# jyf588/SimGAN

Measured on AMD Instinct MI355X. Metric: env-steps/sec of GAIL-dyn PPO update, higher is better.
Workload: dtype f32; 1 GPU; northstar: GAIL-dyn update, T=128 N=512/GPU obs=47 act=12 D-in=86 policy=mlp h64 D h100 ppo_epoch=10 num_mini_batch=1...; optimizer_steps_per_update=2720, parallelism=single GPU

## Files before the change

simgan_amd/_lib.py:

```python
import ctypes as C
import os

import numpy as np

_HERE = os.path.dirname(os.path.abspath(__file__))
LIB_PATH = os.path.join(_HERE, "libsimgan_hip.so")

c_float_p = C.POINTER(C.c_float)
c_i64_p = C.POINTER(C.c_int64)
c_double_p = C.POINTER(C.c_double)
c_u8_p = C.POINTER(C.c_uint8)
c_int_p = C.POINTER(C.c_int)
H = C.c_void_p

F_OBS, F_OBS_FEAT, F_ACTIONS, F_REWARDS, F_VALUE_PREDS, F_RETURNS, F_LOGP, F_MASKS, F_BAD_MASKS, \
    F_ADVANTAGES = range(10)
POLICY_MLP, POLICY_SPLIT, POLICY_GRU = 0, 1, 2
DIST_GAUSSIAN, DIST_CATEGORICAL, DIST_BERNOULLI = 0, 1, 2
CHAIN_INNER_FIRST, CHAIN_LEARNER_FIRST = 0, 1
PROF_DISC_CHAIN, PROF_DISC_WGRAD, PROF_PPO_FWD, PROF_PPO_BWD, PROF_PPO_REDUCE, PROF_RELABEL, PROF_PPO_ADAM = range(7)


class PPOConfig(C.Structure):
    _fields_ = [("clip_param", C.c_float), ("ppo_epoch", C.c_int), ("num_mini_batch", C.c_int),
# ... 100 lines not shown
    "sg_disc_set_expert": (C.c_int, [H, c_float_p, C.c_int64]),
    "sg_disc_update_gail_dyn": (C.c_int, [H, H, C.c_int, c_i64_p, C.c_int64, c_i64_p, C.c_int64, c_float_p, C.c_int64, C.c_uint64,
                                          c_float_p, c_int_p]),
    "sg_disc_update_rows": (C.c_int, [H, c_float_p, C.c_int64, C.c_int, C.c_int, c_i64_p, C.c_int64, c_i64_p, C.c_int64, c_float_p,
                                      C.c_int64, C.c_uint64, c_float_p, c_int_p]),
    "sg_disc_predict_reward": (C.c_int, [H, c_float_p, C.c_int, C.c_float, c_float_p, C.c_float, c_float_p, c_float_p]),
    "sg_disc_predict_prob": (C.c_int, [H, c_float_p, C.c_int, c_float_p]),
    "sg_disc_predict_reward_steps": (C.c_int, [H, H, C.c_float, C.c_float, c_float_p, c_float_p]),
    "sg_disc_grad_pen": (C.c_int, [H, c_float_p, c_float_p, c_float_p, C.c_int, C.c_uint64, c_float_p]),
    "sg_disc_last_draws": (C.c_int, [H, c_i64_p, c_i64_p, c_float_p, c_i64_p]),
    "sg_disc_reset_returns": (C.c_int, [H]),
    "sg_disc_get_returns": (C.c_int, [H, c_float_p, C.c_int, c_int_p]),
    "sg_disc_set_returns": (C.c_int, [H, c_float_p, C.c_int]),
    "sg_disc_relabel_rewards": (C.c_int, [H, H, C.c_float, C.c_float, c_double_p]),
    "sg_disc_relabel_rewards_auto": (C.c_int, [H, H, C.c_float, C.c_double, C.c_int]),
    "sg_disc_set_rms": (C.c_int, [H, c_double_p]),
    "sg_disc_get_scalars": (C.c_int, [H, c_double_p]),
    "sg_disc_diagnostics": (C.c_int, [H, H, C.c_int, c_double_p]),
    "sg_disc_diagnostics_fetch": (C.c_int, [H, C.c_int, c_double_p]),
    "sg_disc_diagnostics_world": (C.c_int, [H, H, C.c_int, c_double_p]),
    "sg_results_publish": (C.c_int, [H, H, H, C.c_int]),
    "sg_results_fetch": (C.c_int, [H, C.c_int, c_double_p]),
    "sg_ctx_profile": (C.c_int, [H, C.c_int]),
    "sg_ctx_profile_read": (C.c_int, [H, C.c_int, c_double_p, c_i64_p]),
    "sg_ctx_profile_reset": (C.c_int, [H]),
    "sg_host_alloc": (C.c_int, [C.c_int64, C.POINTER(C.c_void_p)]),
    "sg_host_free": (C.c_int, [C.c_void_p]),
    "sg_ctx_mark": (C.c_int, [H, c_int_p]),
    "sg_ctx_mark_elapsed": (C.c_int, [H, C.c_int, C.c_int, c_double_p]),
}

TEST_LIB_PATH = os.path.join(_HERE, "libsimgan_hip_test.so")
c_ll_p = C.POINTER(C.c_longlong)
TEST_PROTOTYPES = {
    "sg_test_last_error": (C.c_char_p, []),
    "sg_test_gemm": (C.c_int, [H, C.c_int, C.c_int, C.c_int, C.c_int, c_float_p, c_float_p, c_float_p]),
    "sg_test_gemm_bench": (C.c_int, [H, C.c_int, C.c_int, C.c_int, C.c_int, C.c_int, C.c_int, C.c_int, c_ll_p]),
    "sg_test_mfma_probe": (C.c_int, [H, C.c_int, c_float_p, c_float_p, c_float_p]),
    "sg_test_flag_probe": (C.c_int, [H, C.c_int, C.c_int, C.c_int, C.c_int, c_ll_p, c_float_p]),
    "sg_test_fetch_probe": (C.c_int, [H, C.c_int, C.c_int, C.c_int, c_ll_p]),
    "sg_test_pmc_calibrate": (C.c_int, [H, C.c_int64]),
    "sg_test_pstep_probe": (C.c_int, [H, C.c_int, C.c_int, C.c_int, C.c_int, C.c_int, c_ll_p, c_int_p]),
    "sg_test_graph_state": (C.c_int, [H, H, c_int_p]),
    "sg_test_disc_gathers": (C.c_int, [H, c_ll_p]),
    "sg_test_rng": (C.c_int, [H, C.c_int, C.c_int64, C.c_uint64, C.c_void_p]),
    "sg_test_rng_at": (C.c_int, [H, C.c_int, C.c_int64, C.c_uint64, C.c_uint64, C.c_uint64, C.c_void_p]),
    "sg_test_rng_host": (C.c_int, [C.c_int, C.c_int64, C.c_uint64, C.c_uint64, C.c_uint64, C.c_void_p]),
    "sg_test_kfac_eig": (C.c_int, [H, C.c_int, c_float_p, c_float_p, c_float_p, C.POINTER(C.c_int)]),
    "sg_test_acktr_noise": (C.c_int, [H, C.c_int64, C.c_uint64, C.c_int64, c_float_p]),
    "sg_test_raise_kfac_error": (C.c_int, [H]),
    "sg_test_tear_probe": (C.c_int, [H, C.c_int, C.c_int, C.c_int, c_ll_p]),
    "sg_test_raise_handoff_error": (C.c_int, [H, H]),
    "sg_test_squash": (C.c_int, [c_float_p, c_float_p, C.c_int64]),
}
_TEST_LIB = None

_LIB = None


class SimganHipError(RuntimeError):
    pass


def load():
    global _LIB
    if _LIB is not None:
        return _LIB
    if not os.path.exists(LIB_PATH):
        raise SimganHipError(
            f"{LIB_PATH} not found: the HIP extension is not built. There is no CPU fallback; "
            "run `make -C simgan_amd/csrc` (hipcc, gfx950).")
    lib = C.CDLL(LIB_PATH)
    for name, (res, args) in PROTOTYPES.items():
        fn = getattr(lib, name)
        fn.restype = res
        fn.argtypes = args
    _LIB = lib
    return lib


def check(rc):
    if rc != 0:
        raise SimganHipError(load().sg_last_error().decode(errors="replace"))


def load_test():
    global _TEST_LIB
    if _TEST_LIB is not None:
        return _TEST_LIB
    load()
    if not os.path.exists(TEST_LIB_PATH):
        raise SimganHipError(f"{TEST_LIB_PATH} not found: run `make -C simgan_amd/csrc`")
    lib = C.CDLL(TEST_LIB_PATH)
    for name, (res, args) in TEST_PROTOTYPES.items():
        fn = getattr(lib, name)
        fn.restype = res
        fn.argtypes = args
    _TEST_LIB = lib
    return lib


def check_test(rc):
    if rc != 0:
        raise SimganHipError(load_test().sg_test_last_error().decode(errors="replace"))


# ... 168 lines not shown
```

simgan_amd/csrc/sg_ppo.hip:

```cpp
#include <math.h>
#include <stdlib.h>
#include <string.h>

#include <algorithm>
#include <vector>

#include "sg_common.h"
#include "sg_rng.hpp"
#include "sg_ppo_kernels.hpp"
#include "sg_kfac_host.hpp"
#include "sg_gru_kernels.hpp"

__global__ void k_fill_perm(int64_t* perm, int64_t n, int half_bits, uint64_t key) {
    const int64_t i = (int64_t)blockIdx.x * blockDim.x + threadIdx.x;
    if (i < n) perm[i] = sg_perm_at(i, n, half_bits, key);
}

int sg_fill_perm(sg_ctx* ctx, int64_t* d_perm, int64_t n, uint64_t seed, uint64_t stream_id) {
    const uint64_t key = sg_key(seed, 0x5045524Dull, stream_id);
    hipLaunchKernelGGL(k_fill_perm, dim3((unsigned)((n + 255) / 256)), dim3(256), 0, ctx->stream, d_perm, n,
                       sg_perm_half_bits((uint64_t)n), key);
    SG_CHECK(hipGetLastError());
    return 0;
}
// ... 845 lines not shown
    pa.slabs = a->d_slabs; pa.slab_stride = slab_stride; pa.ldP = ldP;
    pa.st = reinterpret_cast<SgOptState*>(a->d_state); pa.G = G; pa.k1 = 0;
    pa.pair = a->d_pair; pa.Xm = nullptr; pa.MA = nullptr; pa.sym_c = 0.f;
    for (int t = 0; t < 3; ++t) { pa.H1[t] = hX; pa.H2[t] = hX; pa.OUT[t] = hX; }
    pa.X = hX;
    pa.DX[0] = gb + o_dxa; pa.DX[1] = gb + o_dxc;
    pa.wbuf_floats = gw ? 0 : max_trunk_floats(d);

    GruScanArgs tr;
    tr.sr = gb + o_sr; tr.sz = gb + o_sz; tr.sn = gb + o_sn; tr.shn = gb + o_shn; tr.hm = gb + o_hm;
    GruBwdArgs ba;
    ba.g = g; ba.W = pol->d_params + g.off; ba.dxa = gb + o_dxa; ba.dxc = gb + o_dxc; ba.dx_ld = d.ldO;
    ba.sr = tr.sr; ba.sz = tr.sz; ba.sn = tr.sn; ba.shn = tr.shn; ba.hm = tr.hm; ba.T = T; ba.n = per;
    ba.dgi = gb + o_dgi; ba.dgh = gb + o_dgh;
    GruWgradArgs wa;
    wa.g = g; wa.dgi = ba.dgi; wa.dgh = ba.dgh; wa.hm = tr.hm; wa.rows_p = rows_p; wa.KS = KS; wa.partial = gb + o_part;
    const bool gw_scan = sg_gru_force_gw() || sg_gru_scan_lds(g, false) > (size_t)ctx->lds_bytes - 1024 ||
                         sg_gru_bwd_lds(g, false) > (size_t)ctx->lds_bytes - 1024;
    const int n_tiles = (G3 / 16) * (g.Op / 16 + Hp / 16) + 2 * (G3 / 16);
    const size_t lds_b = bwd_lds(MT);
    SgOptState* st = reinterpret_cast<SgOptState*>(a->d_state);

    auto enqueue_steps = [&]() -> int {
        hipLaunchKernelGGL(k_opt_prepare_first, dim3(1), dim3(1), 0, ctx->stream, st);
        for (int e = 0; e < E; ++e) {
            ga.perm = a->d_perms + (size_t)e * N;
            hipLaunchKernelGGL(k_gru_epoch_gather<0>, dim3((unsigned)TN), dim3(64), 0, ctx->stream, ga);
            for (int k = 0; k < S; ++k) {
                const size_t rb = (size_t)k * mb;
                const float* xk = gb + o_x + rb * g.ldO;
                const float* mk = gb + o_mk + rb;
                SG_TRY(sg_gru_forward_launch(ctx, g, pol->d_params + g.off, xk, g.ldO, gb + o_h0 + (size_t)k * per * g.H, mk, T, per,
                                             gb + o_gi, hX, d.ldO, nullptr, &tr));
                pa.ACT = epACT + rb * d.A; pa.SC = epSC + rb;
                pa.k1 = e * S + k + 1;
                if (d.dist == SG_DIST_CATEGORICAL)
                    SG_TRY(ppo_launch(ctx, ppo_bwd_fused_cat_dx_family, "k_ppo_bwd_dist_dx (Categorical)", SG_PROF_PPO_BWD, MT, d, dim3(G, 2),
                                      lds_b, pa, gw));
                else if (d.dist == SG_DIST_BERNOULLI)
                    SG_TRY(ppo_launch(ctx, ppo_bwd_fused_ber_dx_family, "k_ppo_bwd_dist_dx (Bernoulli)", SG_PROF_PPO_BWD, MT, d, dim3(G, 2),
                                      lds_b, pa, gw));
                else
                    SG_TRY(ppo_launch(ctx, ppo_bwd_fused_dx_family, "k_ppo_bwd (fused, with d loss / d h)", SG_PROF_PPO_BWD, MT, d, dim3(G, 2),
                                      lds_b, pa, gw));
                SG_LAUNCH(ctx, SG_PROF_PPO_REDUCE, k_ppo_reduce, dim3(nblk_r), dim3(256), 0, a->d_slabs, G, slab_stride, d.total, a->d_grad,
                          a->d_part);
                ba.masks = mk;
                if (gw_scan) hipLaunchKernelGGL(k_gru_scan_bwd<true>, dim3((per + 15) / 16), dim3(256), sg_gru_bwd_lds(g, true), ctx->stream, ba);
                else hipLaunchKernelGGL(k_gru_scan_bwd<false>, dim3((per + 15) / 16), dim3(256), sg_gru_bwd_lds(g, false), ctx->stream, ba);
                wa.x = xk;
                hipLaunchKernelGGL(k_gru_wgrad<0>, dim3(n_tiles, KS), dim3(64), 0, ctx->stream, wa);
                hipLaunchKernelGGL(k_gru_reduce<0>, dim3(gblocks), dim3(256), 0, ctx->stream, wa.partial, KS, g.total, a->d_grad, d.total,
                                   a->d_part, nblk_r);
                SG_LAUNCH(ctx, SG_PROF_PPO_ADAM, k_ppo_adam, dim3(nblk), dim3(256), 0, pol->d_params, a->d_m, a->d_v, a->d_grad, a->d_part,
                          nblk_r + gblocks, tot_all, st, e * S + k + 1, a->cfg.eps, a->cfg.max_grad_norm, pa.inv_B, a->d_loss_acc);
            }
        }
        hipLaunchKernelGGL(k_opt_commit, dim3(1), dim3(1), 0, ctx->stream, st, E * S);
        SG_CHECK(hipGetLastError());
        return 0;
    };
    const bool use_graph = !ctx->profile && !sg_env_is_off("SG_PPO_GRAPH");
    uint32_t fbits[6];
    const float fv[6] = {a->cfg.clip_param, a->cfg.value_loss_coef, a->cfg.entropy_coef, a->cfg.eps, a->cfg.max_grad_norm, pa.inv_B};
    memcpy(fbits, fv, sizeof fbits);
    const uint64_t key[SG_GRAPH_KEY_WORDS] = {
            (uint64_t)(uintptr_t)a->d_slabs, (uint64_t)(uintptr_t)a->d_stacks, (uint64_t)(uintptr_t)a->d_perms,
            (uint64_t)(uintptr_t)r->d_field[SG_F_OBS], (uint64_t)(uintptr_t)r->d_field[SG_F_ACTIONS],
            (uint64_t)(uintptr_t)r->d_field[SG_F_RETURNS], (uint64_t)(uintptr_t)pol->d_params,
            (uint64_t)TN, ((uint64_t)E << 32) | (uint64_t)M, ((uint64_t)MT << 32) | (uint64_t)G,
            ((uint64_t)fbits[0] << 32) | fbits[1], ((uint64_t)fbits[2] << 32) | fbits[3],
            ((uint64_t)fbits[4] << 32) | fbits[5], (uint64_t)a->cfg.use_clipped_value_loss,
            (uint64_t)(uintptr_t)r->d_field[SG_F_LOGP],
            0x475255ull + (gw ? 8 : 0) + (gw_scan ? 16 : 0) + ((uint64_t)d.dist << 24) + ((uint64_t)N << 32),
            (uint64_t)(uintptr_t)a->d_gru, (uint64_t)(uintptr_t)a->d_h0 ^ ((uint64_t)(uintptr_t)r->d_field[SG_F_MASKS] << 1)};
    SG_TRY(sg_graph_run(ctx, &a->steps_graph, use_graph, key, enqueue_steps));
    SG_CHECK(hipGetLastError());
    a->opt_t += (int64_t)E * S;
    if (!out3) return 0;
    double acc[3];
    SG_TRY(sg_ctx_fetch_f64(ctx, a->d_loss_acc, acc, 3));
    const double nu = (double)E * M;
    for (int i = 0; i < 3; ++i) out3[i] = (float)(acc[i] / nu);
    return 0;
}

#define SG_CNN_MAX_MB 4096
static int cnn_ppo_update(sg_ppo* a, sg_rollout* r, const int64_t* perms, int64_t n_perms, uint64_t seed, float out3[3]) {
    sg_ctx* ctx = a->ctx;
    sg_policy* pol = a->policy;
    const SgPolicyDesc& d = pol->desc;
    const SgCnnDesc& c = pol->cnnd;
    SG_REQUIRE(r->O == d.O && r->A == d.A, "sg_ppo_update: rollout dims (obs %d, act %d) do not match the policy (%d, %d)", r->O, r->A,
               d.O, d.A);
    SG_REQUIRE(!(ctx->use_comm && ctx->world > 1), "sg_ppo_update: PPO on the CNN base runs on one rank (world %d)", ctx->world);
    const int64_t TN = (int64_t)r->T * r->N;
    const int M = a->cfg.num_mini_batch, E = a->cfg.ppo_epoch;
    SG_REQUIRE(TN >= M, "PPO requires the number of processes (%d) * number of steps (%d) = %lld to be greater than "
               "or equal to the number of PPO mini batches (%d).", r->N, r->T, (long long)TN, M);
    SG_REQUIRE(TN < (1ll << 30), "sg_ppo_update: rollout too large");
    const int mb = (int)(TN / M);
    SG_REQUIRE(mb <= SG_CNN_MAX_MB, "sg_ppo_update: a minibatch of %d rows on the CNN base exceeds %d (its activation stacks are "
               "158 KB per row): raise num_mini_batch", mb, SG_CNN_MAX_MB);
    if (perms) {
        SG_REQUIRE(n_perms == (int64_t)E * TN, "sg_ppo_update: perms holds %lld indices, %d epochs x %lld rows need %lld",
                   (long long)n_perms, E, (long long)TN, (long long)E * TN);
        for (int64_t i = 0; i < n_perms; ++i)
            SG_REQUIRE(perms[i] >= 0 && perms[i] < TN, "sg_ppo_update: perms[%lld] = %lld is outside [0, %lld)", (long long)i,
                       (long long)perms[i], (long long)TN);
    }
    SG_CHECK(hipSetDevice(ctx->device));
    SG_TRY(enqueue_adv_stats(ctx, r, a, false));
    SG_TRY(ensure_cap(ctx->stream, &a->d_perms, &a->perms_cap, (int64_t)E * TN));
    a->last_perm_count = (int64_t)E * TN;
    if (perms) {
        SG_CHECK(hipMemcpyAsync(a->d_perms, perms, sizeof(int64_t) * (size_t)E * TN, hipMemcpyHostToDevice, ctx->stream));
        if (!out3) SG_CHECK(hipStreamSynchronize(ctx->stream));
    } else {
        for (int e = 0; e < E; ++e) SG_TRY(sg_fill_perm(ctx, a->d_perms + (size_t)e * TN, TN, seed, (uint64_t)e * 2654435761ull));
    }
    const int hld = d.trunk[0].Pp > 16 ? d.trunk[0].Pp : 16;
    const size_t heads_f = 2 * (size_t)mb * hld, fwd_f = sg_cnn_fwd_floats(c, mb), bwd_f = sg_cnn_bwd_floats(c, mb);
    bool grew = false;
    SG_TRY(ensure_cap(ctx->stream, &a->d_stacks, &a->stacks_cap, heads_f + fwd_f + bwd_f, &grew));
    if (grew) a->cleared.mode = SG_LAYOUT_INVALID;
    float* heads = a->d_stacks;
    float* act = heads + heads_f;
    float* bwd = act + fwd_f;
    hipLaunchKernelGGL(k_zero_f64, dim3(1), dim3(64), 0, ctx->stream, a->d_loss_acc, 4);
    const float inv_B = 1.0f / (float)mb;
    const int nblk = (c.total + 255) / 256;
    SgOptState* st = reinterpret_cast<SgOptState*>(a->d_state);
    const float* obs = r->d_field[SG_F_OBS];

    auto enqueue_steps = [&]() -> int {
        hipLaunchKernelGGL(k_opt_prepare_first, dim3(1), dim3(1), 0, ctx->stream, st);
        for (int e = 0; e < E; ++e)
            for (int k = 0; k < M; ++k) {
                const int64_t* idx = a->d_perms + (size_t)e * TN + (size_t)k * mb;
                SG_TRY(sg_cnn_forward_launch(ctx, pol, obs, idx, mb, act, heads, hld, 0, mb));
                SG_TRY(sg_cnn_backward_launch(ctx, pol, r, obs, idx, mb, act, heads, hld, bwd, a->d_grad, inv_B, a->cfg.clip_param,
                                              a->cfg.value_loss_coef, a->cfg.entropy_coef, a->cfg.use_clipped_value_loss, 0, 0, 0));
                hipLaunchKernelGGL(k_sumsq, dim3(nblk), dim3(256), 0, ctx->stream, a->d_grad, c.total, a->d_part);
                SG_LAUNCH(ctx, SG_PROF_PPO_ADAM, k_ppo_adam, dim3(nblk), dim3(256), 0, pol->d_params, a->d_m, a->d_v, a->d_grad, a->d_part,
                          nblk, c.total, st, e * M + k + 1, a->cfg.eps, a->cfg.max_grad_norm, inv_B, a->d_loss_acc);
            }
        hipLaunchKernelGGL(k_opt_commit, dim3(1), dim3(1), 0, ctx->stream, st, E * M);
        SG_CHECK(hipGetLastError());
        return 0;
    };
    const bool use_graph = !ctx->profile && !sg_env_is_off("SG_PPO_GRAPH");
    uint32_t fbits[6];
    const float fv[6] = {a->cfg.clip_param, a->cfg.value_loss_coef, a->cfg.entropy_coef, a->cfg.eps, a->cfg.max_grad_norm, inv_B};
    memcpy(fbits, fv, sizeof fbits);
    const uint64_t key[SG_GRAPH_KEY_WORDS] = {
            (uint64_t)(uintptr_t)a->d_stacks, (uint64_t)(uintptr_t)a->d_grad, (uint64_t)(uintptr_t)a->d_perms,
            (uint64_t)(uintptr_t)r->d_field[SG_F_OBS], (uint64_t)(uintptr_t)r->d_field[SG_F_ACTIONS],
            (uint64_t)(uintptr_t)r->d_field[SG_F_RETURNS], (uint64_t)(uintptr_t)pol->d_params,
            (uint64_t)TN, ((uint64_t)E << 32) | (uint64_t)M, (uint64_t)mb,
            ((uint64_t)fbits[0] << 32) | fbits[1], ((uint64_t)fbits[2] << 32) | fbits[3],
            ((uint64_t)fbits[4] << 32) | fbits[5], (uint64_t)a->cfg.use_clipped_value_loss,
            (uint64_t)(uintptr_t)r->d_field[SG_F_LOGP],
            0x434E4Eull + ((uint64_t)r->N << 32),
            (uint64_t)(uintptr_t)r->d_field[SG_F_VALUE_PREDS], (uint64_t)(uintptr_t)r->d_field[SG_F_ADVANTAGES]};
    SG_TRY(sg_graph_run(ctx, &a->steps_graph, use_graph, key, enqueue_steps));
    SG_CHECK(hipGetLastError());
    a->opt_t += (int64_t)E * M;
    if (!out3) return 0;
    double acc[3];
    SG_TRY(sg_ctx_fetch_f64(ctx, a->d_loss_acc, acc, 3));
    const double nu = (double)E * M;
    for (int i = 0; i < 3; ++i) out3[i] = (float)(acc[i] / nu);
    return 0;
}

#define SG_A2C_CNN_CHUNK_ROWS 4096
static int a2c_cnn_chunk_rows(int64_t TN) {
    int chunk = SG_A2C_CNN_CHUNK_ROWS;
    if (const char* e = getenv("SG_A2C_CNN_CHUNK_ROWS")) {
        const long v = atol(e);
        if (v >= 1) chunk = (int)std::min<long>(v, SG_CNN_MAX_MB);
    }
    return (int)std::min<int64_t>(chunk, TN);
}

static int a2c_cnn_update(sg_ppo* a, sg_rollout* r, float out3[3]) {
    sg_ctx* ctx = a->ctx;
    sg_policy* pol = a->policy;
    const SgPolicyDesc& d = pol->desc;
    const SgCnnDesc& c = pol->cnnd;
    SG_REQUIRE(r->O == d.O && r->A == d.A, "sg_ppo_update: rollout dims (obs %d, act %d) do not match the policy (%d, %d)", r->O, r->A,
               d.O, d.A);
    SG_REQUIRE(!(ctx->use_comm && ctx->world > 1), "sg_ppo_update: A2C on the CNN base runs on one rank (world %d)", ctx->world);
    const int64_t TN = (int64_t)r->T * r->N;
    SG_REQUIRE(TN > 0 && TN < (1ll << 30), "sg_ppo_update: %lld rollout rows", (long long)TN);
    SG_CHECK(hipSetDevice(ctx->device));
    const int chunk = a2c_cnn_chunk_rows(TN);
// ... 404 lines not shown
    const int nblk_r = (d.total + 8 + SG_PPO_REDUCE_PARAMS - 1) / SG_PPO_REDUCE_PARAMS;
    SgOptState* st = reinterpret_cast<SgOptState*>(a->d_state);

    auto enqueue_steps = [&]() -> int {
        hipLaunchKernelGGL(k_opt_prepare_first, dim3(1), dim3(1), 0, ctx->stream, st);
        for (int e = 0; e < E; ++e) {
            ga.perm = a->d_perms + (size_t)e * TN;
            ga.TN = epoch_rows[e];
            if (ga.TN) hipLaunchKernelGGL(sym ? k_ppo_epoch_gather_sym : k_ppo_epoch_gather, dim3((unsigned)((ga.TN + 63) / 64)), dim3(256), 0,
                                          ctx->stream, ga);
            for (int k = 0; k < M; ++k) {
                const size_t rb = (size_t)step_off[(size_t)e * M + k];
                pa.mb = step_cnt[(size_t)e * M + k];
                pa.X = epX + rb * d.ldO; pa.ACT = epACT + rb * d.A; pa.SC = epSC + rb;
                if (sym) pa.Xm = epXm + rb * d.ldO;
                pa.k1 = e * M + k + 1;
                if (sym) {
                    pa.wbuf_floats = wb_f;
                    SG_TRY(ppo_launch(ctx, ppo_fwd_sym_family, "k_ppo_fwd_sym", SG_PROF_PPO_FWD, MT, d, dim3(G, 3), lds_f, pa, gw));
                    pa.wbuf_floats = wb_b;
                    SG_TRY(ppo_launch(ctx, ppo_bwd_sym_family, "k_ppo_bwd_sym", SG_PROF_PPO_BWD, MT, d, dim3(G, 3), lds_b, pa, gw));
                } else if (pair) {
                    pa.wbuf_floats = wb_f;
                    SG_TRY(ppo_launch(ctx, ppo_pair_family, "k_ppo_pair", SG_PROF_PPO_BWD, MT, d, dim3(3 * G), lds_fc, pa, false));
                } else if (crit_first) {
                    pa.wbuf_floats = wb_f;
                    SG_TRY(ppo_launch(ctx, ppo_fwd_critic_family, "k_ppo_fwd_critic", SG_PROF_PPO_FWD, MT, d, dim3(G, d.n_trunks),
                                      lds_fc > lds_f ? lds_fc : lds_f, pa, false));
                    pa.wbuf_floats = wb_b;
                    SG_TRY(ppo_launch(ctx, ppo_bwd_family, "k_ppo_bwd", SG_PROF_PPO_BWD, MT, d, dim3(G, d.n_trunks - 1), lds_b, pa,
                                      false));
                } else if (fused) {
                    pa.wbuf_floats = wb_f;
                    if (d.dist == SG_DIST_CATEGORICAL)
                        SG_TRY(ppo_launch(ctx, ppo_bwd_fused_cat_family, "k_ppo_bwd (fused, categorical)", SG_PROF_PPO_BWD, MT, d, dim3(G, d.n_trunks), lds_b, pa, gw));
                    else if (d.dist == SG_DIST_BERNOULLI)
                        SG_TRY(ppo_launch(ctx, ppo_bwd_fused_ber_family, "k_ppo_bwd (fused, Bernoulli)", SG_PROF_PPO_BWD, MT, d, dim3(G, d.n_trunks), lds_b, pa, gw));
                    else
                        SG_TRY(ppo_launch(ctx, ppo_bwd_fused_family, "k_ppo_bwd (fused)", SG_PROF_PPO_BWD, MT, d, dim3(G, d.n_trunks), lds_b, pa, gw));
                } else {
                    pa.wbuf_floats = wb_f;
                    SG_TRY(ppo_launch(ctx, ppo_fwd_family, "k_ppo_fwd", SG_PROF_PPO_FWD, MT, d, dim3(G, d.n_trunks), lds_f, pa, gw));
                    pa.wbuf_floats = wb_b;
                    SG_TRY(ppo_launch(ctx, ppo_bwd_family, "k_ppo_bwd", SG_PROF_PPO_BWD, MT, d, dim3(G, d.n_trunks), lds_b, pa, gw));
                }
                if (sym) SG_LAUNCH(ctx, SG_PROF_PPO_REDUCE, k_ppo_reduce_sym, dim3(nblk_r), dim3(256), 0, a->d_slabs, G, slab_stride,
                                   d.total, a->d_grad, a->d_part, d.trunk[0].off, d.trunk[0].off + d.trunk[0].ex);
                else SG_LAUNCH(ctx, SG_PROF_PPO_REDUCE, k_ppo_reduce, dim3(nblk_r), dim3(256), 0, a->d_slabs, G, slab_stride,
                               d.total, a->d_grad, a->d_part);
                if (ctx->use_comm) {
                    SG_TRY(sg_comm_allreduce_f32(ctx, a->d_grad, d.total + 8));
                    hipLaunchKernelGGL(k_sumsq, dim3(nblk), dim3(256), 0, ctx->stream, a->d_grad, d.total, a->d_part);
                }
                SG_LAUNCH(ctx, SG_PROF_PPO_ADAM, sym ? k_ppo_adam_sym : k_ppo_adam, dim3(nblk), dim3(256), 0, a->policy->d_params, a->d_m,
                          a->d_v, a->d_grad, a->d_part, ctx->use_comm ? nblk : nblk_r, d.total, st, e * M + k + 1, a->cfg.eps,
                          a->cfg.max_grad_norm, pa.inv_B, a->d_loss_acc);
            }
        }
        hipLaunchKernelGGL(k_opt_commit, dim3(1), dim3(1), 0, ctx->stream, st, E * M);
        return 0;
    };
    const bool comm_ok = !ctx->use_comm || (sg_comm_graph_ok(ctx) && !sg_env_is_off("SG_PPO_GRAPH_COMM"));
    const bool use_graph = comm_ok && !owned && !ctx->profile && !sg_env_is_off("SG_PPO_GRAPH");
    uint32_t fbits[6];
    const float fv[6] = {a->cfg.clip_param, a->cfg.value_loss_coef, a->cfg.entropy_coef, a->cfg.eps, a->cfg.max_grad_norm, pa.inv_B};
    memcpy(fbits, fv, sizeof fbits);
    uint32_t cbits;
    memcpy(&cbits, &a->sym_coef, sizeof cbits);
    const uint64_t key[SG_GRAPH_KEY_WORDS] = {
            (uint64_t)(uintptr_t)a->d_slabs, (uint64_t)(uintptr_t)a->d_stacks, (uint64_t)(uintptr_t)a->d_perms,
            (uint64_t)(uintptr_t)r->d_field[SG_F_OBS], (uint64_t)(uintptr_t)r->d_field[SG_F_ACTIONS],
            (uint64_t)(uintptr_t)r->d_field[SG_F_RETURNS], (uint64_t)(uintptr_t)a->policy->d_params,
            (uint64_t)TN, ((uint64_t)E << 32) | (uint64_t)M, ((uint64_t)MT << 32) | (uint64_t)G,
            ((uint64_t)fbits[0] << 32) | fbits[1], ((uint64_t)fbits[2] << 32) | fbits[3],
            ((uint64_t)fbits[4] << 32) | fbits[5], (uint64_t)a->cfg.use_clipped_value_loss,
            (uint64_t)(uintptr_t)r->d_field[SG_F_LOGP], 0x50504full + (fused ? 1 : 0) + (ctx->use_comm ? 2 : 0) + (crit_first ? 4 : 0) + (gw ? 8 : 0) + (pair ? 16 : 0) + (sg_comm_peer_on(ctx) ? 32 : 0) + (sym ? 64 : 0) + ((uint64_t)sg_comm_peer_generation(ctx) << 32),
            sym ? (uint64_t)(uintptr_t)a->d_mrows : 0, sym ? (uint64_t)cbits : 0};
    SG_TRY(sg_graph_run(ctx, &a->steps_graph, use_graph, key, enqueue_steps));
    SG_CHECK(hipGetLastError());
    a->opt_t += (int64_t)E * M;
    if (!out3) return 0;
    double acc[3];
    SG_TRY(sg_ctx_fetch_f64(ctx, a->d_loss_acc, acc, 3));
    if (pair && (acc[0] != acc[0] || acc[1] != acc[1] || acc[2] != acc[2])) {
        unsigned err = 0;
        SG_COPY_SYNC(ctx, &err, a->d_pair + SG_PAIR_ERR_WORD, sizeof err, hipMemcpyDeviceToHost);
        if (err) {
            SG_CHECK(hipMemsetAsync(a->d_pair + SG_PAIR_ERR_WORD, 0, sizeof err, ctx->stream));
            a->self_wait_failed = true;
            SG_REQUIRE(false, "sg_ppo_update: a workgroup of k_ppo_pair waited %d s for its partner's words and gave "
                       "up (the policy's state is undefined; SG_PPO_PAIR=0 runs the multi-launch step)", (int)(SG_PAIR_TIMEOUT_TICKS / 100000000ll));
        }
    }
    const double nu = (double)E * M;
    for (int i = 0; i < 3; ++i) out3[i] = (float)(acc[i] / nu);
    return 0;
}

__global__ void k_publish(double* dst, const double* d_acc, const double* d_scal, const double* p_acc, double n_d, double n_p,
                          const unsigned* d_err, const unsigned* a_err, const unsigned* peer_err) {
    const int t = threadIdx.x;
    if (t < 3) dst[t] = d_acc ? d_acc[t] : 0.0;
    else if (t < 8) dst[t] = d_scal ? d_scal[t - 3] : 0.0;
    else if (t < 11) dst[t] = p_acc ? p_acc[t - 8] : 0.0;
    else if (t == 11) dst[t] = n_d;
    else if (t == 12) dst[t] = n_p;
    else if (t == 13) dst[t] = d_err ? (double)*d_err : 0.0;
// ... 58 lines not shown
```

simgan_amd/csrc/sg_ppo_kernels.hpp:

```cpp
#pragma once
#include "sg_common.h"
#include "sg_thin.hpp"

struct PpoArgs {
    SgPolicyDesc d;
    const float* params;
    const float* X;
    const float* ACT;
    const float* SC;
    int sc_stride;
    int mb, mbp;
    float inv_B;
    float clip, vcoef, ecoef;
    int use_clipped;
    float* H1[3];
    float* H2[3];
    float* OUT[3];
    float* slabs;
    int slab_stride;
    int ldP;
    int wbuf_floats;
    SgOptState* st;
    int k1, G;
    unsigned* pair;
// ... 571 lines not shown
    if (PAIR && pair_failed && tid == 0) {
        atomicOr(a.pair + SG_PAIR_ERR_WORD, 1u);
        slab[d.total + 1] = __builtin_nanf("");
    }
}

template <int MT, int KO, int KH, bool FUSED = false, bool GW = false, bool DX = false>
__global__ __launch_bounds__(512) void k_ppo_bwd(PpoArgs a) {
    sg_ppo_bwd_body<MT, KO, KH, FUSED, GW, false, false, false, DX>(a, blockIdx.y, blockIdx.x);
}
template <int MT, bool GW, int DIST>
__global__ __launch_bounds__(512) void k_ppo_bwd_dist(PpoArgs a) {
    sg_ppo_bwd_body<MT, 0, 0, true, GW, false, false, false, false, DIST>(a, blockIdx.y, blockIdx.x);
}
template <int MT, bool GW, int DIST>
__global__ __launch_bounds__(512) void k_ppo_bwd_dist_dx(PpoArgs a) {
    sg_ppo_bwd_body<MT, 0, 0, true, GW, false, false, false, true, DIST>(a, blockIdx.y, blockIdx.x);
}
template <int MT, int KO, int KH, bool GW = false>
__global__ __launch_bounds__(512) void k_ppo_bwd_sym(PpoArgs a) {
    sg_ppo_bwd_body<MT, KO, KH, false, GW, false, true>(a, blockIdx.y, blockIdx.x);
}

template <int MT, int KO, int KH, bool GW = false>
__global__ __launch_bounds__(512) void k_a2c_bwd(PpoArgs a) {
    sg_ppo_bwd_body<MT, KO, KH, false, GW, false, false, true>(a, blockIdx.y, blockIdx.x);
}
template <int MT, bool GW>
__global__ __launch_bounds__(512) void k_a2c_bwd_dx(PpoArgs a) {
    sg_ppo_bwd_body<MT, 0, 0, false, GW, false, false, true, true>(a, blockIdx.y, blockIdx.x);
}
template <int MT, bool GW, int DIST>
__global__ __launch_bounds__(512) void k_a2c_bwd_dist(PpoArgs a) {
    sg_ppo_bwd_body<MT, 0, 0, false, GW, false, false, true, false, DIST>(a, blockIdx.y, blockIdx.x);
}
template <int MT, bool GW, int DIST>
__global__ __launch_bounds__(512) void k_a2c_bwd_dist_dx(PpoArgs a) {
    sg_ppo_bwd_body<MT, 0, 0, false, GW, false, false, true, true, DIST>(a, blockIdx.y, blockIdx.x);
}

template <int MT, int KO, int KH>
__global__ __launch_bounds__(512) void k_ppo_pair(PpoArgs a) {
    const int bx = (int)blockIdx.x / 3, t = (int)blockIdx.x - 3 * bx;
    sg_ppo_bwd_body<MT, KO, KH, true, false, true>(a, t, bx);
}

template <int MT, int KO, int KH>
__global__ __launch_bounds__(512) void k_ppo_fwd_critic(PpoArgs a) {
    if (blockIdx.y == 0) sg_ppo_bwd_body<MT, KO, KH, true>(a, a.d.n_trunks - 1, blockIdx.x);
    else sg_ppo_fwd_body<MT, KO, KH>(a, blockIdx.y - 1, blockIdx.x);
}

#define SG_PPO_REDUCE_PARAMS 64
template <bool SYM, bool ACC = false>
__device__ __forceinline__ void sg_ppo_reduce_body(const float* slabs, int n_slabs_, int slab_stride, int total,
                                                   float* grad, float* part, int lo2, int hi2, int acc = 0) {
    __shared__ float red[4][64];
    const int lane = threadIdx.x & 63, wave = threadIdx.x >> 6;
    const int i = blockIdx.x * SG_PPO_REDUCE_PARAMS + lane;
    const int n_slabs = (SYM && i >= lo2 && i < hi2) ? 2 * n_slabs_ : n_slabs_;
    float g = 0.f;
    if (i < total + 8) {
        for (int s0 = wave; s0 < n_slabs; s0 += 64) {
            float t[16];
#pragma unroll
            for (int u = 0; u < 16; ++u) {
                const int sidx = s0 + 4 * u;
                t[u] = slabs[(size_t)(sidx < n_slabs ? sidx : s0) * slab_stride + i];
            }
#pragma unroll
            for (int u = 0; u < 16; ++u) g += (s0 + 4 * u < n_slabs) ? t[u] : 0.f;
        }
    }
    red[wave][lane] = g;
    __syncthreads();
    if (wave == 0) {
        g = (red[0][lane] + red[1][lane]) + (red[2][lane] + red[3][lane]);
        if (ACC && acc && i < total + 8) g += grad[i];
        if (i < total + 8) grad[i] = g;
        float sq = (i < total) ? g * g : 0.f;
        sq = sg_wave_sum(sq);
        if (lane == 0) part[blockIdx.x] = sq;
    }
}
__global__ __launch_bounds__(256) void k_ppo_reduce(const float* slabs, int n_slabs, int slab_stride, int total,
                                                    float* grad, float* part) {
    sg_ppo_reduce_body<false>(slabs, n_slabs, slab_stride, total, grad, part, 0, 0);
}
__global__ __launch_bounds__(256) void k_ppo_reduce_sym(const float* slabs, int n_slabs, int slab_stride, int total,
                                                        float* grad, float* part, int lo2, int hi2) {
    sg_ppo_reduce_body<true>(slabs, n_slabs, slab_stride, total, grad, part, lo2, hi2);
}
__global__ __launch_bounds__(256) void k_a2c_reduce(const float* slabs, int n_slabs, int slab_stride, int total,
                                                    float* grad, float* part, int acc) {
    sg_ppo_reduce_body<false, true>(slabs, n_slabs, slab_stride, total, grad, part, 0, 0, acc);
}

__global__ void k_opt_prepare_first(SgOptState* st) { sg_opt_prepare(st, st->t0 + 1); }

__global__ __launch_bounds__(256) void k_sumsq(const float* grad, int total, float* part) {
    const int i = blockIdx.x * blockDim.x + threadIdx.x;
    float sq = (i < total) ? grad[i] * grad[i] : 0.f;
    sq = sg_wave_sum(sq);
    __shared__ float ws[4];
    if ((threadIdx.x & 63) == 0) ws[threadIdx.x >> 6] = sq;
    __syncthreads();
    if (threadIdx.x == 0) part[blockIdx.x] = ws[0] + ws[1] + ws[2] + ws[3];
}

template <int NL>
__device__ __forceinline__ void sg_ppo_adam_body(float* params, float* m, float* v, const float* grad,
                                                 const float* part, int n_part, int total,
                                                 const SgOptState* st, int k1, float eps, float max_norm,
                                                 float inv_mb, double* loss_acc) {
    __shared__ float s_coef;
    const int t = st->t0 + k1;
    const float s_step_size = st->step_size2[t & 1], s_bc2_sqrt = st->bc2_sqrt2[t & 1];
    __shared__ float s_ws[4];
    {
        float s = 0.f;
        for (int j = threadIdx.x; j < n_part; j += 256) s += part[j];
        s = sg_wave_sum(s);
        if ((threadIdx.x & 63) == 0) s_ws[threadIdx.x >> 6] = s;
    }
    __syncthreads();
    if (threadIdx.x == 0) {
        const float norm = sqrtf((s_ws[0] + s_ws[1]) + (s_ws[2] + s_ws[3]));
        float coef = max_norm / (norm + 1e-6f);
        s_coef = coef > 1.f ? 1.f : coef;
    }
    __syncthreads();
    const int i = blockIdx.x * blockDim.x + threadIdx.x;
    if (i < total) {
        const float g = grad[i] * s_coef;
        float mi = m[i], vi = v[i];
        mi = mi + (g - mi) * (float)(1.0 - 0.9);
        vi = vi * (float)0.999 + (float)(1.0 - 0.999) * g * g;
        const float denom = sqrtf(vi) / s_bc2_sqrt + eps;
        params[i] = params[i] - s_step_size * (mi / denom);
        m[i] = mi;
        v[i] = vi;
    }
    if (blockIdx.x == 0 && threadIdx.x < NL)
        loss_acc[threadIdx.x] += (double)(grad[total + threadIdx.x] * inv_mb);
    if (blockIdx.x == 0 && threadIdx.x == 64) sg_opt_prepare(const_cast<SgOptState*>(st), t + 1);
}
__global__ __launch_bounds__(256) void k_ppo_adam(float* params, float* m, float* v, const float* grad,
                                                  const float* part, int n_part, int total,
                                                  const SgOptState* st, int k1, float eps, float max_norm,
                                                  float inv_mb, double* loss_acc) {
    sg_ppo_adam_body<3>(params, m, v, grad, part, n_part, total, st, k1, eps, max_norm, inv_mb, loss_acc);
}
__global__ __launch_bounds__(256) void k_ppo_adam_sym(float* params, float* m, float* v, const float* grad,
                                                      const float* part, int n_part, int total,
                                                      const SgOptState* st, int k1, float eps, float max_norm,
                                                      float inv_mb, double* loss_acc) {
    sg_ppo_adam_body<4>(params, m, v, grad, part, n_part, total, st, k1, eps, max_norm, inv_mb, loss_acc);
}

__global__ __launch_bounds__(256) void k_a2c_rmsprop(float* params, float* sq, const float* grad, const float* part, int n_part,
                                                     int total, const SgOptState* st, float alpha, float one_m_alpha, float eps,
                                                     float max_norm, float inv_b, double* loss_acc) {
    __shared__ float s_coef;
    __shared__ float s_ws[4];
    {
        float s = 0.f;
        for (int j = threadIdx.x; j < n_part; j += 256) s += part[j];
        s = sg_wave_sum(s);
        if ((threadIdx.x & 63) == 0) s_ws[threadIdx.x >> 6] = s;
    }
    __syncthreads();
    if (threadIdx.x == 0) {
        const float norm = sqrtf((s_ws[0] + s_ws[1]) + (s_ws[2] + s_ws[3]));
        const float coef = max_norm / (norm + 1e-6f);
        s_coef = coef > 1.f ? 1.f : coef;
    }
    __syncthreads();
    const int i = blockIdx.x * blockDim.x + threadIdx.x;
    if (i < total) {
        const float g = grad[i] * s_coef;
        const float s = sq[i] * alpha + one_m_alpha * g * g;
        params[i] = params[i] + (-st->lr) * (g / (sqrtf(s) + eps));
        sq[i] = s;
    }
    if (blockIdx.x == 0 && threadIdx.x < 3) loss_acc[threadIdx.x] += (double)(grad[total + threadIdx.x] * inv_b);
}

__global__ __launch_bounds__(1024) void k_adv_stats(const float* ret, const float* vpred, int64_t n, float* adv,
                                                    double* stats ,
                                                    int pass) {
    __shared__ double ws[16];
    __shared__ double s_mean;
    const int tid = threadIdx.x;
    if (pass == 0) {
        double s = 0.0;
        for (int64_t i = tid; i < n; i += blockDim.x) {
            const float a = ret[i] - vpred[i];
            adv[i] = a;
            s += (double)a;
        }
        s = sg_wave_sum(s);
        if ((tid & 63) == 0) ws[tid >> 6] = s;
        __syncthreads();
        if (tid == 0) {
            double t = 0.0;
            for (int w = 0; w < (int)(blockDim.x >> 6); ++w) t += ws[w];
            stats[0] = t;
            stats[2] = (double)n;
        }
    } else if (pass == 1) {
        if (tid == 0) s_mean = (double)(float)(stats[0] / stats[2]);
        __syncthreads();
        const double mean = s_mean;
        double s = 0.0;
        for (int64_t i = tid; i < n; i += blockDim.x) {
            const double dd = (double)adv[i] - mean;
            s += dd * dd;
        }
        s = sg_wave_sum(s);
        if ((tid & 63) == 0) ws[tid >> 6] = s;
        __syncthreads();
        if (tid == 0) {
            double t = 0.0;
            for (int w = 0; w < (int)(blockDim.x >> 6); ++w) t += ws[w];
            stats[1] = t;
        }
    } else {
        const float mean = (float)(stats[0] / stats[2]);
        const float sd = (float)sqrt(stats[1] / (stats[2] - 1.0));
        for (int64_t i = tid + (int64_t)blockIdx.x * blockDim.x; i < n; i += (int64_t)gridDim.x * blockDim.x)
            adv[i] = (adv[i] - mean) / (sd + 1e-5f);
    }
}
```

simgan_amd/csrc/sg_test_api.h:

```cpp
#pragma once
#include <stdint.h>

#include "../../include/simgan_hip.h"

#ifdef __cplusplus
extern "C" {
#endif
SG_API const char *sg_test_last_error(void);
SG_API int sg_test_gemm(sg_ctx *ctx, int mode, int M, int N, int K, const float *A, const float *B, float *C);
SG_API int sg_test_gemm_bench(sg_ctx *ctx, int mode, int MT, int K, int Np, int threads, int iters, int epi, long long *cycles);
SG_API int sg_test_mfma_probe(sg_ctx *ctx, int abid, const float *a, const float *b, float *d);
SG_API int sg_test_flag_probe(sg_ctx *ctx, int mode, int np, int nc, int words, long long *stamps, float *sums);
SG_API int sg_test_fetch_probe(sg_ctx *ctx, int n_blocks, int waves, int mode, long long *out);
SG_API int sg_test_pstep_probe(sg_ctx *ctx, int mode, int S, int NW, int cyc_phase, int cyc_w, long long *stamps, int *err4);
SG_API int sg_test_pmc_calibrate(sg_ctx *ctx, int64_t mbytes);
SG_API int sg_test_graph_state(sg_ppo *a, sg_disc *d, int out[2]);
SG_API int sg_test_disc_gathers(sg_disc *d, long long *out);
SG_API int sg_test_tear_probe(sg_ctx *ctx, int mode, int pairs4, int iters, long long *out4);
SG_API int sg_test_rng(sg_ctx *ctx, int kind, int64_t n, uint64_t seed, void *out);
SG_API int sg_test_rng_at(sg_ctx *ctx, int kind, int64_t n, uint64_t seed, uint64_t stream, uint64_t ctr0, void *out);
SG_API int sg_test_rng_host(int kind, int64_t n, uint64_t seed, uint64_t stream, uint64_t ctr0, void *out);
SG_API int sg_test_raise_handoff_error(sg_disc *d, sg_ppo *a);
SG_API int sg_test_kfac_eig(sg_ctx *ctx, int n, const float *A, float *Q, float *d, int *sweeps);
SG_API int sg_test_acktr_noise(sg_ctx *ctx, int64_t n, uint64_t seed, int64_t update, float *out);
SG_API int sg_test_raise_kfac_error(sg_ppo *a);
SG_API int sg_test_squash(const float *in, float *out, int64_t n);
#ifdef __cplusplus
}
#endif
```

Before: 2.560 million env-steps/s.

## Hoist loads ahead of grad-norm reduction in PPO Adam and batch slab reduce loads

The Adam kernels now issue their per-element loads (grad, moments, params, loss accumulator) and the first batch of partial-norm loads before the block reduction and barriers, so global memory latency overlaps the norm computation. The optimizer-state prepare moves into an extra trailing block to take it off block 0's critical path. The slab reduction uses templated batches of up to 64 outstanding loads with byte-offset addressing and a wave-uniform wave index. Register pressure rises, and a read/write hazard on the optimizer state across blocks could appear if other blocks read st while the last block updates it.

```diff
diff --git a/simgan_amd/_lib.py b/simgan_amd/_lib.py
--- a/simgan_amd/_lib.py
+++ b/simgan_amd/_lib.py
@@ -176,6 +176,9 @@
     "sg_test_tear_probe": (C.c_int, [H, C.c_int, C.c_int, C.c_int, c_ll_p]),
     "sg_test_raise_handoff_error": (C.c_int, [H, H]),
     "sg_test_squash": (C.c_int, [c_float_p, c_float_p, C.c_int64]),
+    "sg_test_ppo_reduce": (C.c_int, [H, C.c_int, c_float_p, C.c_int, C.c_int, C.c_int, C.c_int, C.c_int, C.c_int, c_float_p, c_float_p]),
+    "sg_test_ppo_adam": (C.c_int, [H, C.c_int, c_float_p, c_float_p, c_float_p, c_float_p, c_float_p, C.c_int, C.c_int, C.c_int, C.c_int,
+                                   C.c_float, C.c_float, C.c_float, C.c_float, c_double_p, c_float_p]),
 }
 _TEST_LIB = None
 
diff --git a/simgan_amd/csrc/sg_ppo.hip b/simgan_amd/csrc/sg_ppo.hip
--- a/simgan_amd/csrc/sg_ppo.hip
+++ b/simgan_amd/csrc/sg_ppo.hip
@@ -921,7 +921,7 @@
                 hipLaunchKernelGGL(k_gru_wgrad<0>, dim3(n_tiles, KS), dim3(64), 0, ctx->stream, wa);
                 hipLaunchKernelGGL(k_gru_reduce<0>, dim3(gblocks), dim3(256), 0, ctx->stream, wa.partial, KS, g.total, a->d_grad, d.total,
                                    a->d_part, nblk_r);
-                SG_LAUNCH(ctx, SG_PROF_PPO_ADAM, k_ppo_adam, dim3(nblk), dim3(256), 0, pol->d_params, a->d_m, a->d_v, a->d_grad, a->d_part,
+                SG_LAUNCH(ctx, SG_PROF_PPO_ADAM, k_ppo_adam, dim3(nblk + 1), dim3(256), 0, pol->d_params, a->d_m, a->d_v, a->d_grad, a->d_part,
                           nblk_r + gblocks, tot_all, st, e * S + k + 1, a->cfg.eps, a->cfg.max_grad_norm, pa.inv_B, a->d_loss_acc);
             }
         }
@@ -1011,7 +1011,7 @@
                 SG_TRY(sg_cnn_backward_launch(ctx, pol, r, obs, idx, mb, act, heads, hld, bwd, a->d_grad, inv_B, a->cfg.clip_param,
                                               a->cfg.value_loss_coef, a->cfg.entropy_coef, a->cfg.use_clipped_value_loss, 0, 0, 0));
                 hipLaunchKernelGGL(k_sumsq, dim3(nblk), dim3(256), 0, ctx->stream, a->d_grad, c.total, a->d_part);
-                SG_LAUNCH(ctx, SG_PROF_PPO_ADAM, k_ppo_adam, dim3(nblk), dim3(256), 0, pol->d_params, a->d_m, a->d_v, a->d_grad, a->d_part,
+                SG_LAUNCH(ctx, SG_PROF_PPO_ADAM, k_ppo_adam, dim3(nblk + 1), dim3(256), 0, pol->d_params, a->d_m, a->d_v, a->d_grad, a->d_part,
                           nblk, c.total, st, e * M + k + 1, a->cfg.eps, a->cfg.max_grad_norm, inv_B, a->d_loss_acc);
             }
         hipLaunchKernelGGL(k_opt_commit, dim3(1), dim3(1), 0, ctx->stream, st, E * M);
@@ -1522,7 +1522,7 @@
                     SG_TRY(sg_comm_allreduce_f32(ctx, a->d_grad, d.total + 8));
                     hipLaunchKernelGGL(k_sumsq, dim3(nblk), dim3(256), 0, ctx->stream, a->d_grad, d.total, a->d_part);
                 }
-                SG_LAUNCH(ctx, SG_PROF_PPO_ADAM, sym ? k_ppo_adam_sym : k_ppo_adam, dim3(nblk), dim3(256), 0, a->policy->d_params, a->d_m,
+                SG_LAUNCH(ctx, SG_PROF_PPO_ADAM, sym ? k_ppo_adam_sym : k_ppo_adam, dim3(nblk + 1), dim3(256), 0, a->policy->d_params, a->d_m,
                           a->d_v, a->d_grad, a->d_part, ctx->use_comm ? nblk : nblk_r, d.total, st, e * M + k + 1, a->cfg.eps,
                           a->cfg.max_grad_norm, pa.inv_B, a->d_loss_acc);
             }
diff --git a/simgan_amd/csrc/sg_ppo_kernels.hpp b/simgan_amd/csrc/sg_ppo_kernels.hpp
--- a/simgan_amd/csrc/sg_ppo_kernels.hpp
+++ b/simgan_amd/csrc/sg_ppo_kernels.hpp
@@ -647,31 +647,44 @@
 }
 
 #define SG_PPO_REDUCE_PARAMS 64
+template <int NB>
+__device__ __forceinline__ float sg_ppo_reduce_batch(const char* col, unsigned lane_off, int s0, int n_issue, int n_sum,
+                                                     size_t stride_bytes, float g) {
+    float t[NB];
+#pragma unroll
+    for (int u = 0; u < NB; ++u) {
+        const int sidx = s0 + 4 * u;
+        t[u] = *reinterpret_cast<const float*>(col + (size_t)(sidx < n_issue ? sidx : s0) * stride_bytes + lane_off);
+    }
+    __builtin_amdgcn_sched_barrier(0);
+#pragma unroll
+    for (int u = 0; u < NB; ++u) g += (s0 + 4 * u < n_sum) ? t[u] : 0.f;
+    return g;
+}
 template <bool SYM, bool ACC = false>
 __device__ __forceinline__ void sg_ppo_reduce_body(const float* slabs, int n_slabs_, int slab_stride, int total,
                                                    float* grad, float* part, int lo2, int hi2, int acc = 0) {
     __shared__ float red[4][64];
-    const int lane = threadIdx.x & 63, wave = threadIdx.x >> 6;
-    const int i = blockIdx.x * SG_PPO_REDUCE_PARAMS + lane;
+    const int lane = threadIdx.x & 63, wave = __builtin_amdgcn_readfirstlane(threadIdx.x >> 6);
+    const int i0 = blockIdx.x * SG_PPO_REDUCE_PARAMS, i = i0 + lane;
     const int n_slabs = (SYM && i >= lo2 && i < hi2) ? 2 * n_slabs_ : n_slabs_;
-    float g = 0.f;
+    const int n_issue = (SYM && i0 < hi2 && i0 + SG_PPO_REDUCE_PARAMS > lo2) ? 2 * n_slabs_ : n_slabs_;
+    float g = 0.f, g_old = 0.f;
+    if (ACC && acc && wave == 0 && i < total + 8) g_old = grad[i];
     if (i < total + 8) {
-        for (int s0 = wave; s0 < n_slabs; s0 += 64) {
-            float t[16];
-#pragma unroll
-            for (int u = 0; u < 16; ++u) {
-                const int sidx = s0 + 4 * u;
-                t[u] = slabs[(size_t)(sidx < n_slabs ? sidx : s0) * slab_stride + i];
-            }
-#pragma unroll
-            for (int u = 0; u < 16; ++u) g += (s0 + 4 * u < n_slabs) ? t[u] : 0.f;
-        }
+        const char* col = reinterpret_cast<const char*>(slabs) + (size_t)i0 * sizeof(float);
+        const unsigned lane_off = (unsigned)lane * (unsigned)sizeof(float);
+        const size_t sb = (size_t)slab_stride * sizeof(float);
+        int s0 = wave;
+        for (; s0 + 4 * 32 < n_issue; s0 += 4 * 64) g = sg_ppo_reduce_batch<64>(col, lane_off, s0, n_issue, n_slabs, sb, g);
+        if (s0 + 4 * 16 < n_issue) g = sg_ppo_reduce_batch<32>(col, lane_off, s0, n_issue, n_slabs, sb, g);
+        else if (s0 < n_issue) g = sg_ppo_reduce_batch<16>(col, lane_off, s0, n_issue, n_slabs, sb, g);
     }
     red[wave][lane] = g;
     __syncthreads();
     if (wave == 0) {
         g = (red[0][lane] + red[1][lane]) + (red[2][lane] + red[3][lane]);
-        if (ACC && acc && i < total + 8) g += grad[i];
+        if (ACC && acc && i < total + 8) g += g_old;
         if (i < total + 8) grad[i] = g;
         float sq = (i < total) ? g * g : 0.f;
         sq = sg_wave_sum(sq);
@@ -703,42 +716,70 @@
     if (threadIdx.x == 0) part[blockIdx.x] = ws[0] + ws[1] + ws[2] + ws[3];
 }
 
+#define SG_ADAM_PART_BATCH 4
+__device__ __forceinline__ void sg_part_request(float (&pj)[SG_ADAM_PART_BATCH], const float* part, int n_part, int j0) {
+#pragma unroll
+    for (int u = 0; u < SG_ADAM_PART_BATCH; ++u) {
+        const int j = j0 + 256 * u;
+        pj[u] = part[j < n_part ? j : 0];
+    }
+}
+__device__ __forceinline__ float sg_part_add(const float (&pj)[SG_ADAM_PART_BATCH], int n_part, int j0, float s) {
+#pragma unroll
+    for (int u = 0; u < SG_ADAM_PART_BATCH; ++u) s += (j0 + 256 * u < n_part) ? pj[u] : 0.f;
+    return s;
+}
 template <int NL>
 __device__ __forceinline__ void sg_ppo_adam_body(float* params, float* m, float* v, const float* grad,
                                                  const float* part, int n_part, int total,
                                                  const SgOptState* st, int k1, float eps, float max_norm,
                                                  float inv_mb, double* loss_acc) {
     __shared__ float s_coef;
+    __shared__ float s_ws[4];
+    const int tid = threadIdx.x, i = blockIdx.x * 256 + tid;
+    const bool loss_lane = blockIdx.x == 0 && tid < NL;
+    if (blockIdx.x == gridDim.x - 1) {
+        if (tid == 0) sg_opt_prepare(const_cast<SgOptState*>(st), st->t0 + k1 + 1);
+        return;
+    }
+    float pj[SG_ADAM_PART_BATCH];
+    sg_part_request(pj, part, n_part, tid);
+    float gi = 0.f, mi = 0.f, vi = 0.f, pi = 0.f, lt = 0.f;
+    double la = 0.0;
+    if (i < total) { gi = grad[i]; mi = m[i]; vi = v[i]; pi = params[i]; }
+    if (loss_lane) { lt = grad[total + tid]; la = loss_acc[tid]; }
+    __builtin_amdgcn_sched_barrier(0);
+    const float4 sc = *reinterpret_cast<const float4*>(st->step_size2);
     const int t = st->t0 + k1;
-    const float s_step_size = st->step_size2[t & 1], s_bc2_sqrt = st->bc2_sqrt2[t & 1];
-    __shared__ float s_ws[4];
+    const float s_step_size = (t & 1) ? sc.y : sc.x, s_bc2_sqrt = (t & 1) ? sc.w : sc.z;
     {
-        float s = 0.f;
-        for (int j = threadIdx.x; j < n_part; j += 256) s += part[j];
+        float s = sg_part_add(pj, n_part, tid, 0.f);
+        for (int j0 = tid + 256 * SG_ADAM_PART_BATCH; j0 < n_part; j0 += 256 * SG_ADAM_PART_BATCH) {
+            sg_part_request(pj, part, n_part, j0);
+            s = sg_part_add(pj, n_part, j0, s);
+        }
         s = sg_wave_sum(s);
-        if ((threadIdx.x & 63) == 0) s_ws[threadIdx.x >> 6] = s;
-    }
-    __syncthreads();
-    if (threadIdx.x == 0) {
+        if ((tid & 63) == 0) s_ws[tid >> 6] = s;
+    }
+    __syncthreads();
+    if (tid == 0) {
         const float norm = sqrtf((s_ws[0] + s_ws[1]) + (s_ws[2] + s_ws[3]));
         float coef = max_norm / (norm + 1e-6f);
         s_coef = coef > 1.f ? 1.f : coef;
     }
     __syncthreads();
-    const int i = blockIdx.x * blockDim.x + threadIdx.x;
+    asm volatile("" : "+v"(gi), "+v"(mi), "+v"(vi), "+v"(pi), "+v"(lt), "+v"(la));
     if (i < total) {
-        const float g = grad[i] * s_coef;
-        float mi = m[i], vi = v[i];
+        const float g = gi * s_coef;
         mi = mi + (g - mi) * (float)(1.0 - 0.9);
         vi = vi * (float)0.999 + (float)(1.0 - 0.999) * g * g;
         const float denom = sqrtf(vi) / s_bc2_sqrt + eps;
-        params[i] = params[i] - s_step_size * (mi / denom);
+        params[i] = pi - s_step_size * (mi / denom);
         m[i] = mi;
         v[i] = vi;
     }
-    if (blockIdx.x == 0 && threadIdx.x < NL)
-        loss_acc[threadIdx.x] += (double)(grad[total + threadIdx.x] * inv_mb);
-    if (blockIdx.x == 0 && threadIdx.x == 64) sg_opt_prepare(const_cast<SgOptState*>(st), t + 1);
+    if (loss_lane)
+        loss_acc[tid] = la + (double)(lt * inv_mb);
 }
 __global__ __launch_bounds__(256) void k_ppo_adam(float* params, float* m, float* v, const float* grad,
                                                   const float* part, int n_part, int total,
@@ -758,27 +799,41 @@
                                                      float max_norm, float inv_b, double* loss_acc) {
     __shared__ float s_coef;
     __shared__ float s_ws[4];
+    const int tid = threadIdx.x, i = blockIdx.x * 256 + tid;
+    const bool loss_lane = blockIdx.x == 0 && tid < 3;
+    float pj[SG_ADAM_PART_BATCH];
+    sg_part_request(pj, part, n_part, tid);
+    float gi = 0.f, si = 0.f, pi = 0.f, lt = 0.f;
+    double la = 0.0;
+    if (i < total) { gi = grad[i]; si = sq[i]; pi = params[i]; }
+    if (loss_lane) { lt = grad[total + tid]; la = loss_acc[tid]; }
+    __builtin_amdgcn_sched_barrier(0);
+    const float lr = st->lr;
+    __builtin_amdgcn_sched_barrier(0);
     {
-        float s = 0.f;
-        for (int j = threadIdx.x; j < n_part; j += 256) s += part[j];
+        float s = sg_part_add(pj, n_part, tid, 0.f);
+        for (int j0 = tid + 256 * SG_ADAM_PART_BATCH; j0 < n_part; j0 += 256 * SG_ADAM_PART_BATCH) {
+            sg_part_request(pj, part, n_part, j0);
+            s = sg_part_add(pj, n_part, j0, s);
+        }
         s = sg_wave_sum(s);
-        if ((threadIdx.x & 63) == 0) s_ws[threadIdx.x >> 6] = s;
-    }
-    __syncthreads();
-    if (threadIdx.x == 0) {
+        if ((tid & 63) == 0) s_ws[tid >> 6] = s;
+    }
+    __syncthreads();
+    if (tid == 0) {
         const float norm = sqrtf((s_ws[0] + s_ws[1]) + (s_ws[2] + s_ws[3]));
         const float coef = max_norm / (norm + 1e-6f);
         s_coef = coef > 1.f ? 1.f : coef;
     }
     __syncthreads();
-    const int i = blockIdx.x * blockDim.x + threadIdx.x;
+    asm volatile("" : "+v"(gi), "+v"(si), "+v"(pi), "+v"(lt), "+v"(la));
     if (i < total) {
-        const float g = grad[i] * s_coef;
-        const float s = sq[i] * alpha + one_m_alpha * g * g;
-        params[i] = params[i] + (-st->lr) * (g / (sqrtf(s) + eps));
+        const float g = gi * s_coef;
+        const float s = si * alpha + one_m_alpha * g * g;
+        params[i] = pi + (-lr) * (g / (sqrtf(s) + eps));
         sq[i] = s;
     }
-    if (blockIdx.x == 0 && threadIdx.x < 3) loss_acc[threadIdx.x] += (double)(grad[total + threadIdx.x] * inv_b);
+    if (loss_lane) loss_acc[tid] = la + (double)(lt * inv_b);
 }
 
 __global__ __launch_bounds__(1024) void k_adv_stats(const float* ret, const float* vpred, int64_t n, float* adv,
diff --git a/simgan_amd/csrc/sg_test_api.h b/simgan_amd/csrc/sg_test_api.h
--- a/simgan_amd/csrc/sg_test_api.h
+++ b/simgan_amd/csrc/sg_test_api.h
@@ -25,6 +25,11 @@
 SG_API int sg_test_acktr_noise(sg_ctx *ctx, int64_t n, uint64_t seed, int64_t update, float *out);
 SG_API int sg_test_raise_kfac_error(sg_ppo *a);
 SG_API int sg_test_squash(const float *in, float *out, int64_t n);
+SG_API int sg_test_ppo_reduce(sg_ctx *ctx, int mode, const float *slabs, int n_slabs, int slab_stride, int total, int lo2, int hi2,
+                              int acc, float *grad_inout, float *part_out);
+SG_API int sg_test_ppo_adam(sg_ctx *ctx, int sym, float *params, float *m, float *v, const float *grad, const float *part, int n_part,
+                            int total, int t0, int k1, float lr, float eps, float max_norm, float inv_mb, double *loss_acc_inout,
+                            float *state_out);
 #ifdef __cplusplus
 }
 #endif
```

After: 2.584 million env-steps/s, median of 6. About the same (+0.9%).
